# ocramz/rp-tree

Measured on AMD Instinct MI355X. Metric: forest-build vectors/s (1000000 x 128 dense f64, 32 trees; projection mode mfma = RPT_PROJ_MFMA, the API default RPT_PROJ_AUTO on f64 data is the exact-order kernel timed in `other_projection_mode`); kNN queries/s and recall@10 in `knn` / `recall_at_10`, higher is better.
Workload: dtype f64; 1 GPU; C2: 1000000 x 128 f64 two-Gaussian mixture, 32-tree forest, minLeaf 128, maxDepth 13, pnz 0.4746, k=10, 10000 queries; trees sharded 32/GPU, X replicated; projection_mode=mfma

## Files before the change

rp-tree_amd/csrc/split.hip:

```cpp
#include <algorithm>
#include <chrono>
#include <cmath>
#include <cstdio>
#include <cstdlib>
#include <functional>
#include <limits>
#include <list>

#include "common.h"
#include "codes.h"

extern "C" __device__ unsigned int __ockl_median3_u32(unsigned int, unsigned int, unsigned int);

namespace rpt {
namespace {

constexpr int kSmallCap = 4096;
constexpr int kNB = 1024;
constexpr int kSample = 1024;
constexpr int kDelta = 80;
constexpr int kChunk = 4096;
constexpr int kPad = 0x7fffffff;

template <class TK>
// ... 3004 lines not shown
  if (!(kmin < kmax)) return false;
  const double inv = 1024.0 / ((double)kmax - (double)kmin);
  auto sub_of = [&](TK k) -> int {
    const int b = (int)(((double)k - (double)kmin) * inv);
    return b > 1023 ? 1023 : b;
  };
  for (int i = tid; i < cMid; i += 256) atomicAdd(&sel_hist[sub_of(skey[i])], 1);
  __syncthreads();
  const int kk = a.nh - a.cL;
  if (wave == 0) {
    int c[16], tot = 0;
#pragma unroll
    for (int q = 0; q < 16; ++q) {
      c[q] = sel_hist[lane * 16 + q];
      tot += c[q];
    }
    int inc = tot;
    for (int o = 1; o < 64; o <<= 1) {
      const int p = __shfl_up(inc, o);
      if (lane >= o) inc += p;
    }
    int run = inc - tot;
    if (kk >= run && kk < inc) {
#pragma unroll
      for (int q = 0; q < 16; ++q) {
        if (kk >= run && kk < run + c[q]) {
          sel_misc[0] = lane * 16 + q;
          sel_misc[1] = run;
          sel_misc[2] = c[q];
        }
        run += c[q];
      }
    }
  }
  __syncthreads();
  const int sstar = sel_misc[0], below = sel_misc[1], mc = sel_misc[2];
  if (mc > 128) return false;
  unsigned long long lowmax = 0ULL, highmin = ~0ULL;
  for (int i = tid; i < cMid; i += 256) {
    const TK k = skey[i];
    const int sb = sub_of(k);
    if (sb == sstar) {
      sel_cand[atomicAdd(&sel_misc[3], 1)] = i;
    } else {
      const unsigned long long o = ord_of(k);
      if (sb < sstar) lowmax = o > lowmax ? o : lowmax;
      else highmin = o < highmin ? o : highmin;
    }
  }
  for (int o = 32; o > 0; o >>= 1) {
    const unsigned long long p = __shfl_xor(lowmax, o), q = __shfl_xor(highmin, o);
    lowmax = p > lowmax ? p : lowmax;
    highmin = q < highmin ? q : highmin;
  }
  __syncthreads();
  if (lane == 0) {
    sel_red[wave] = lowmax;
    sel_red[4 + wave] = highmin;
  }
  __syncthreads();
  uint16_t* no = A.node_of + (int64_t)t * N;
  unsigned long long mn[2] = {~0ULL, ~0ULL}, mx[2] = {0ULL, 0ULL};
  const bool feed_next = A.has_next && cMid * 4 >= a.n;
  auto place = [&](int id, int side) {
    no[id] = (uint16_t)(2 * j + side);
    if (feed_next) {
      const unsigned long long o = ord_of(mid_next_key(A, t, id));
      mn[side] = o < mn[side] ? o : mn[side];
      mx[side] = o > mx[side] ? o : mx[side];
    }
  };
  if (wave == 0) {
    for (int w = 0; w < 4; ++w) {
      lowmax = sel_red[w] > lowmax ? sel_red[w] : lowmax;
      highmin = sel_red[4 + w] < highmin ? sel_red[4 + w] : highmin;
    }
    Keys<TK> K{A.P + (int64_t)t * A.L * N, N, A.level, nullptr};
    TK k[2];
    int id[2];
#pragma unroll
    for (int r = 0; r < 2; ++r) {
      const int q = r * 64 + lane;
      const int i = q < mc ? sel_cand[q] : -1;
      id[r] = i >= 0 ? sid[i] : kPad;
      k[r] = i >= 0 ? skey[i] : pos_inf<TK>();
    }
    wave_bitonic_fast<TK, 2>(k, id, K);
    const int n = a.n, nh = a.nh;
    const int il = nh > 0 ? nh - 1 : 0, ih = nh + 1 < n ? nh + 1 : n - 1;
    const int ql = il - a.cL, qh = ih - a.cL;
    TK vthr = (TK)0, vlo = (TK)0, vhi = (TK)0;
    int have = 0;
#pragma unroll
    for (int r = 0; r < 2; ++r) {
      const int q = below + r * 64 + lane;
      if (r * 64 + lane < mc) {
        place(id[r], q >= kk);
        if (q == kk) {
          vthr = k[r];
          have |= 1;
        }
        if (q == ql) {
          vlo = k[r];
          have |= 2;
        }
        if (q == qh) {
          vhi = k[r];
          have |= 4;
        }
      }
    }
    const unsigned long long b1 = __ballot(have & 1), b2 = __ballot(have & 2), b4 = __ballot(have & 4);
    const TK tthr = __shfl(vthr, __ffsll((long long)b1) - 1);
    TK tlo, thi;
    if (b2) tlo = __shfl(vlo, __ffsll((long long)b2) - 1);
    else if (ql < 0) tlo = ord_to(a.maxL, TK());
    else tlo = ord_to(lowmax, TK());
    if (b4) thi = __shfl(vhi, __ffsll((long long)b4) - 1);
    else if (qh >= cMid) thi = ord_to(a.minR, TK());
    else thi = ord_to(highmin, TK());
    if (lane == 0) {
      const int64_t h = (int64_t)t * A.nodes + A.heap0 + j;
      A.thr[h] = (double)tthr;
      A.mglo[h] = (double)tlo;
      A.mghi[h] = (double)thi;
      if (nh > 0 && !(tlo < tthr)) atomicAdd(A.tie_count, 1ULL);
    }
  }
  for (int i = tid; i < cMid; i += 256) {
    const int sb = sub_of(skey[i]);
    if (sb != sstar) place(sid[i], sb > sstar);
  }
  if (feed_next) {
    for (int sd = 0; sd < 2; ++sd) {
      unsigned long long x = mn[sd], y = mx[sd];
      for (int o = 32; o > 0; o >>= 1) {
        const unsigned long long p = __shfl_xor(x, o), q = __shfl_xor(y, o);
        x = p < x ? p : x;
        y = q > y ? q : y;
      }
      if (lane == 0) {
        if (x != ~0ULL) atomicMin(&A.cmin_next[(int64_t)t * 2 * M + 2 * j + sd], x);
        if (y != 0ULL) atomicMax(&A.cmax_next[(int64_t)t * 2 * M + 2 * j + sd], y);
      }
    }
  }
  return true;
}

constexpr int kMidWaveLds = 512;

template <class TK>
__global__ __launch_bounds__(256) void stream_mid(const MidArgs<TK> A, int npb, int wave_max,
                                                  int use_select ) {
  extern __shared__ __attribute__((aligned(16))) unsigned char smem[];
  __shared__ int sbig[4];
  const int w = threadIdx.x >> 6, lane = threadIdx.x & 63, t = blockIdx.y;
  const int jw = blockIdx.x * npb + w;
  int big = 0;
  if (w < npb && jw < A.M) {
    const SNode<TK> a = A.nd[(int64_t)t * A.M + jw];
    if (a.cMid > wave_max) {
      if (npb > 1 && a.cMid <= kMidWaveLds)
        mid_lds_path<TK, true>(A, a, t, jw, smem + (size_t)w * kMidWaveLds * (sizeof(TK) + 4));
      else
        big = a.cMid <= kSmallCap;
    } else if (a.cMid > 0) {
      mid_wave_path<TK>(A, a, t, jw, lane);
    }
  }
  if (lane == 0) sbig[w] = big;
  __syncthreads();
  for (int q = 0; q < npb; ++q) {
    if (!sbig[q]) continue;
    const int j = blockIdx.x * npb + q;
    const SNode<TK> a = A.nd[(int64_t)t * A.M + j];
    if (use_select && mid_select_path<TK>(A, a, t, j, smem)) {
      __syncthreads();
      continue;
    }
    __syncthreads();
    mid_lds_path<TK, false>(A, a, t, j, smem);
    __syncthreads();
  }
}

constexpr int kPermChunk = 8192;
template <class TK>
__global__ __launch_bounds__(kStreamThreads) void stream_to_perm(
    const uint16_t* __restrict__ node_of, int64_t N, int levels, int64_t per,
    unsigned int* __restrict__ gcur, int32_t* __restrict__ perm,
    const unsigned int* __restrict__ abort) {
  constexpr int EPT = kPermChunk / kStreamThreads;
  __shared__ unsigned int cnt[2 * kStreamMaxNodes];
  __shared__ int gb[2 * kStreamMaxNodes], noff[2 * kStreamMaxNodes];
  __shared__ int sid[kPermChunk];
  __shared__ unsigned short sj[kPermChunk];
  __shared__ unsigned int wsum[kStreamThreads / 64];
  if (*abort) return;
  const int t = blockIdx.y;
  const int M = 1 << levels;
  const int lane = threadIdx.x & 63, wave = threadIdx.x >> 6;
  const uint16_t* no = node_of + (int64_t)t * N;
  int32_t* pm = perm + (int64_t)t * N;
  const int64_t i0 = (int64_t)blockIdx.x * per, i1 = i0 + per < N ? i0 + per : N;
  for (int j = threadIdx.x; j < M; j += kStreamThreads) {
    int64_t off = 0, n = N;
    for (int b = levels - 1; b >= 0; --b) {
      const int64_t nh = n >> 1;
      if ((j >> b) & 1) {
        off += nh;
        n -= nh;
      } else {
        n = nh;
      }
    }
    noff[j] = (int)off;
  }
  for (int64_t c0 = i0; c0 < i1; c0 += kPermChunk) {
    const int cn = (int)(i1 - c0 < kPermChunk ? i1 - c0 : kPermChunk);
    for (int j = threadIdx.x; j < M; j += kStreamThreads) cnt[j] = 0;
    __syncthreads();
    unsigned int pk[EPT];
#pragma unroll
    for (int e = 0; e < EPT; ++e) {
      const int k = e * kStreamThreads + threadIdx.x;
      pk[e] = 0xffffffffu;
      if (k < cn) {
        const unsigned int j = no[c0 + k];
        pk[e] = (j << 16) | atomicAdd(&cnt[j], 1u);
      }
    }
    __syncthreads();
    unsigned int v0 = 0, v1 = 0;
    const int j0 = 2 * threadIdx.x, j1 = j0 + 1;
    if (j0 < M) v0 = cnt[j0];
    if (j1 < M) v1 = cnt[j1];
    unsigned int inc = v0 + v1;
    for (int o = 1; o < 64; o <<= 1) {
      const unsigned int u = __shfl_up(inc, o);
      if (lane >= o) inc += u;
    }
    if (lane == 63) wsum[wave] = inc;
    __syncthreads();
    unsigned int pre = inc - (v0 + v1);
    for (int w = 0; w < wave; ++w) pre += wsum[w];
    if (j0 < M) {
      cnt[j0] = pre;
      gb[j0] = v0 ? noff[j0] + (int)atomicAdd(&gcur[(int64_t)t * M + j0], v0) - (int)pre : 0;
    }
    if (j1 < M) {
      cnt[j1] = pre + v0;
      gb[j1] = v1 ? noff[j1] + (int)atomicAdd(&gcur[(int64_t)t * M + j1], v1) - (int)(pre + v0) : 0;
    }
    __syncthreads();
#pragma unroll
    for (int e = 0; e < EPT; ++e)
      if (pk[e] != 0xffffffffu) {
        const unsigned int j = pk[e] >> 16, r = pk[e] & 0xffffu;
        const int sl = (int)(cnt[j] + r);
        sid[sl] = (int)(c0 + e * kStreamThreads + threadIdx.x);
        sj[sl] = (unsigned short)j;
      }
    __syncthreads();
    for (int k = threadIdx.x; k < cn; k += kStreamThreads) pm[gb[sj[k]] + k] = sid[k];
    __syncthreads();
  }
}

__device__ inline double sample_value(double v) { return v; }
__device__ inline double sample_value(float v) { return (double)v; }
__device__ inline double sample_value(uint16_t v) {
  return (double)__uint_as_float((unsigned int)v << 16);
}
template <class TIn, class TK>
__global__ __launch_bounds__(256) void sample_range_kernel(const TIn* __restrict__ X, int64_t stride,
                                                           int S, int d, const double* __restrict__ R,
                                                           int C, int L, int Lc,
                                                           unsigned long long* __restrict__ mm) {
  constexpr int CG = 16, KCH = 128;
  __shared__ __attribute__((aligned(16))) double rl[KCH * CG];
  const int c0 = blockIdx.x * CG;
  const int si = blockIdx.y * 256 + threadIdx.x;
  const bool live = si < S;
  const TIn* xr = X + (int64_t)(live ? si : 0) * stride * d;
  double acc[CG];
#pragma unroll
  for (int c = 0; c < CG; ++c) acc[c] = 0.0;
  for (int k0 = 0; k0 < d; k0 += KCH) {
    const int kn = d - k0 < KCH ? d - k0 : KCH;
    __syncthreads();
    for (int i = threadIdx.x; i < kn * CG; i += 256) {
      const int c = i / kn, k = i % kn;
      rl[k * CG + c] = c0 + c < C ? R[(int64_t)(c0 + c) * d + k0 + k] : 0.0;
    }
    __syncthreads();
    int k = 0;
    for (; k + 16 <= kn; k += 16) {
      TIn xv[16];
#pragma unroll
      for (int u = 0; u < 16; ++u) xv[u] = xr[k0 + k + u];
#pragma unroll
      for (int u = 0; u < 16; ++u) {
        const double x = sample_value(xv[u]);
#pragma unroll
        for (int c = 0; c < CG; ++c) acc[c] = __builtin_fma(x, rl[(k + u) * CG + c], acc[c]);
      }
    }
    for (; k < kn; ++k) {
      const double x = sample_value(xr[k0 + k]);
#pragma unroll
      for (int c = 0; c < CG; ++c) acc[c] = __builtin_fma(x, rl[k * CG + c], acc[c]);
    }
  }
  unsigned long long mn = ~0ULL, mx = 0ULL;
#pragma unroll
  for (int c = 0; c < CG; ++c) {
    const TK v = (TK)acc[c];
    if (live && c0 + c < C && (c0 + c) % L < Lc && v == v) {
      const unsigned long long o = ord_of(v);
      mn = o < mn ? o : mn;
      mx = o > mx ? o : mx;
    }
  }
  for (int o = 32; o > 0; o >>= 1) {
    const unsigned long long a = __shfl_xor(mn, o), b = __shfl_xor(mx, o);
    mn = a < mn ? a : mn;
    mx = b > mx ? b : mx;
  }
  if ((threadIdx.x & 63) == 0 && mn <= mx) {
    atomicMin(&mm[0], mn);
    atomicMax(&mm[1], mx);
  }
}

template <class TK>
__global__ __launch_bounds__(256) void pcode_range_kernel(const TK* __restrict__ P, int64_t N, int L,
                                                          int Lc, unsigned long long* mm) {
  const int c = blockIdx.x;
  if (c % L >= Lc) return;
  const TK* col = P + (int64_t)c * N;
  const int64_t m = N < 4096 ? N : 4096;
  unsigned long long mn = ~0ULL, mx = 0ULL;
  for (int64_t i = threadIdx.x; i < m; i += 256) {
    const unsigned long long o = ord_of(col[i * N / m]);
    mn = o < mn ? o : mn;
    mx = o > mx ? o : mx;
  }
  for (int o = 32; o > 0; o >>= 1) {
    const unsigned long long a = __shfl_xor(mn, o), b = __shfl_xor(mx, o);
    mn = a < mn ? a : mn;
    mx = b > mx ? b : mx;
  }
  if ((threadIdx.x & 63) == 0) {
    atomicMin(mm, mn);
    atomicMax(mm + 1, mx);
  }
}

template <class TK>
__global__ __launch_bounds__(256) void pcode_kernel(const TK* __restrict__ P, int64_t N, int L, int Lc,
                                                    const unsigned long long* __restrict__ mm,
                                                    uint16_t* __restrict__ codes) {
  const int c = blockIdx.y;
  if (c % L >= Lc) return;
  const CodeGeo<TK> g = code_geo<TK>(mm[0], mm[1]);
  const TK* col = P + (int64_t)c * N;
  uint16_t* out = codes + (int64_t)c * N;
  const int64_t n8 = N / 8;
  for (int64_t i = (int64_t)blockIdx.x * 256 + threadIdx.x; i < n8; i += (int64_t)gridDim.x * 256) {
    struct alignas(16) V8 { uint16_t v[8]; } o;
#pragma unroll
    for (int e = 0; e < 8; ++e) o.v[e] = code_of(col[i * 8 + e], g);
    *reinterpret_cast<V8*>(out + i * 8) = o;
  }
  if (blockIdx.x == 0)
    for (int64_t i = n8 * 8 + threadIdx.x; i < N; i += 256) out[i] = code_of(col[i], g);
}

__global__ void build_init_kernel(double* thr, double* mglo, double* mghi, int64_t n,
                                  unsigned long long* counters , unsigned int* sflags ) {
  const double nan = __longlong_as_double(0x7ff8000000000000LL);
  for (int64_t i = blockIdx.x * (int64_t)blockDim.x + threadIdx.x; i < n;
       i += (int64_t)gridDim.x * blockDim.x) {
    thr[i] = nan;
    mglo[i] = nan;
    mghi[i] = nan;
  }
  if (blockIdx.x == 0 && threadIdx.x < 2) counters[threadIdx.x] = 0ULL;
  if (blockIdx.x == 0 && threadIdx.x < 4) sflags[threadIdx.x] = 0u;
}

__global__ void stream_init_kernel(unsigned long long* cmin, unsigned long long* cmax, int T,
                                   unsigned int* poolcur, int npool) {
  for (int i = blockIdx.x * blockDim.x + threadIdx.x; i < T; i += gridDim.x * blockDim.x) {
    cmin[i] = ~0ULL;
    cmax[i] = 0ULL;
  }
  for (int i = blockIdx.x * blockDim.x + threadIdx.x; i < npool; i += gridDim.x * blockDim.x)
    poolcur[i] = 0u;
}

struct GSeg {
  int64_t off;
  int32_t n;
  int32_t t;
  int32_t heap;
  int32_t nh_rel, il_rel, ih_rel;
};

template <class TK>
__global__ __launch_bounds__(256) void gsort_chunk_kernel(int32_t* buf, int64_t N, const TK* P,
                                                          int L, int level,
                                                          const GSeg* __restrict__ gs,
                                                          const int32_t* tb) {
  extern __shared__ __attribute__((aligned(16))) unsigned char smem[];
  const GSeg g = gs[blockIdx.y];
  const int64_t c0 = (int64_t)blockIdx.x * kSmallCap;
  if (c0 >= g.n) return;
  const int n = (int)((g.n - c0) < kSmallCap ? (g.n - c0) : kSmallCap);
  const int np = next_pow2(n);
  TK* skey = reinterpret_cast<TK*>(smem);
  int* sid = reinterpret_cast<int*>(smem + (size_t)np * sizeof(TK));
  Keys<TK> K{P + (int64_t)g.t * L * N, N, level, tb ? tb + (int64_t)g.t * N : nullptr};
  int32_t* s = buf + g.off + c0;
  for (int i = threadIdx.x; i < np; i += blockDim.x) {
    if (i < n) {
      const int id = s[i];
      sid[i] = id;
      skey[i] = K.key(id);
    } else {
      sid[i] = kPad;
      skey[i] = pos_inf<TK>();
    }
  }
  __syncthreads();
  lds_bitonic(skey, sid, np, K);
  for (int i = threadIdx.x; i < n; i += blockDim.x) s[i] = sid[i];
}

template <class TK>
__global__ __launch_bounds__(256) void gsort_merge_kernel(const int32_t* __restrict__ in,
                                                          int32_t* __restrict__ out, int64_t N,
                                                          const TK* P, int L, int level,
                                                          const GSeg* __restrict__ gs, int64_t w,
                                                          const int32_t* tb) {
  const GSeg g = gs[blockIdx.y];
  const int64_t i = (int64_t)blockIdx.x * 256 + threadIdx.x;
  if (i >= g.n) return;
  Keys<TK> K{P + (int64_t)g.t * L * N, N, level, tb ? tb + (int64_t)g.t * N : nullptr};
  const int32_t* s = in + g.off;
  const int id = s[i];
  const int64_t run = i / w, pair0 = (run & ~1LL) * w;
  const bool in_a = (run & 1) == 0;
  const int64_t o0 = in_a ? pair0 + w : pair0;
  int64_t olen = g.n - o0;
  if (olen > w) olen = w;
  int64_t rank = 0;
  if (olen > 0) {
    const TK key = K.key(id);
    int64_t lo = 0, hi = olen;
    while (lo < hi) {
      const int64_t mid = (lo + hi) >> 1;
      const int oid = s[o0 + mid];
      if (K.less(K.key(oid), oid, key, id)) lo = mid + 1;
      else hi = mid;
    }
    rank = lo;
  }
  const int64_t own = in_a ? i - pair0 : i - (pair0 + w);
  out[g.off + pair0 + own + rank] = id;
}

__global__ void gsort_copy_kernel(const int32_t* __restrict__ in, int32_t* __restrict__ out,
                                  const GSeg* __restrict__ gs) {
  const GSeg g = gs[blockIdx.y];
  const int64_t i = (int64_t)blockIdx.x * 256 + threadIdx.x;
  if (i < g.n) out[g.off + i] = in[g.off + i];
}

template <class TK>
__global__ void gsort_emit_kernel(const int32_t* __restrict__ buf, int64_t N, const TK* P, int L,
                                  int level, const GSeg* __restrict__ gs, int G,
                                  const NodeAux* aux_of , const int* aux_idx,
                                  double* thr, double* mglo, double* mghi, int64_t nodes,
                                  unsigned long long* tie_count) {
  const int gi = blockIdx.x * blockDim.x + threadIdx.x;
  if (gi >= G) return;
  const GSeg g = gs[gi];
  if (g.heap < 0) return;
  const TK* Pl = P + ((int64_t)g.t * L + level) * N;
  const int64_t h = (int64_t)g.t * nodes + g.heap;
  const TK vthr = Pl[buf[g.off + g.nh_rel]];
  TK vlo, vhi;
  if (g.il_rel >= 0) vlo = Pl[buf[g.off + g.il_rel]];
  else vlo = ord_to(aux_of[aux_idx[gi]].maxL, TK());
  if (g.ih_rel >= 0) vhi = Pl[buf[g.off + g.ih_rel]];
  else vhi = ord_to(aux_of[aux_idx[gi]].minR, TK());
  thr[h] = (double)vthr;
  mglo[h] = (double)vlo;
  mghi[h] = (double)vhi;
  if (!(vlo < vthr)) atomicAdd(tie_count, 1ULL);
}

template <class TK>
int32_t gsort(rpt_ctx* ctx, int32_t* buf, int32_t* tmp, int64_t N, const TK* P, int L, int level,
              const std::vector<GSeg>& list, DevBuf<GSeg>& dlist, const int32_t* tb) {
  if (list.empty()) return RPT_OK;
  RPT_TRY(dlist.alloc(list.size()));
  RPT_HIP(hipMemcpyAsync(dlist.p, list.data(), list.size() * sizeof(GSeg), hipMemcpyHostToDevice,
                         ctx->stream));
  RPT_HIP(stream_sync(ctx->stream));
  int64_t nmax = 0;
  for (const GSeg& g : list) nmax = g.n > nmax ? g.n : nmax;
  const unsigned G = (unsigned)list.size();
  const size_t smem = (size_t)kSmallCap * (sizeof(TK) + 4);
  hipLaunchKernelGGL(gsort_chunk_kernel<TK>, dim3((unsigned)((nmax + kSmallCap - 1) / kSmallCap), G),
                     dim3(256), smem, ctx->stream, buf, N, P, L, level, dlist.p, tb);
  int32_t* a = buf;
  int32_t* b = tmp;
  for (int64_t w = kSmallCap; w < nmax; w *= 2) {
    hipLaunchKernelGGL(gsort_merge_kernel<TK>, dim3((unsigned)((nmax + 255) / 256), G), dim3(256),
                       0, ctx->stream, a, b, N, P, L, level, dlist.p, w, tb);
    std::swap(a, b);
  }
  if (a != buf)
    hipLaunchKernelGGL(gsort_copy_kernel, dim3((unsigned)((nmax + 255) / 256), G), dim3(256), 0,
                       ctx->stream, a, buf, dlist.p);
  RPT_HIP(hipGetLastError());
  return RPT_OK;
}

static double now_ms() {
  return std::chrono::duration<double, std::milli>(std::chrono::steady_clock::now().time_since_epoch()).count();
}
#define HT(label) do { if (ctx->opt.debug_host) { (void)stream_sync(ctx->stream); double t__ = now_ms(); fprintf(stderr, "host %-28s %8.3f ms\n", label, t__ - ht_last); ht_last = t__; } } while (0)

template <class TK>
int32_t build_forest_t(rpt_ctx* ctx, const rpt_dataset* ds, rpt_forest* f, int32_t mode,
                       bool no_stream = false) {
  double ht_last = now_ms();
  const int64_t N = f->n;
  const int T = f->T, L = f->L;
  hipStream_t st = ctx->stream;
  f->mode = mode;
  ctx->last_csub_redo = ctx->last_csub_bad = 0;

  int Lused = 0;
  {
    int64_t n = N;
    for (int l = 0; l < L; ++l) {
      if (n > (int64_t)f->min_leaf) Lused = l + 1;
      n -= n / 2;
    }
  }
  DevBuf<unsigned long long> counters;
  DevBuf<unsigned int> sflags;
  RPT_TRY(counters.alloc(2));
  RPT_TRY(sflags.alloc(4));
  hipLaunchKernelGGL(build_init_kernel, dim3(256), dim3(256), 0, st, f->thr.p, f->mglo.p, f->mghi.p,
                     (int64_t)T * f->nodes, counters.p, sflags.p);
  if (N == 0) return RPT_OK;
  if (Lused == 0) {
    hipLaunchKernelGGL(iota_kernel, dim3(1024), dim3(256), 0, st, f->perm.p, N, T);
    RPT_HIP(hipGetLastError());
    return RPT_OK;
  }

  RPT_TRY(f->proj.alloc((size_t)T * L * N * sizeof(TK)));
  TK* P = reinterpret_cast<TK*>(f->proj.p);
  const int stream_cap = ctx->opt.stream_maxnodes > 0
                             ? (int)(ctx->opt.stream_maxnodes < kStreamMaxNodes ? ctx->opt.stream_maxnodes
                                                                                : kStreamMaxNodes)
                             : (N / 1024 > kSmallCap ? 1024 : 512);
  int Lc = 0;
  if (N >= 2048 && !no_stream && !ctx->opt.no_stream) {
    int64_t nmin = N;
    while (Lc < Lused && nmin > (int64_t)f->min_leaf && (1 << Lc) <= stream_cap) {
      ++Lc;
      nmin /= 2;
    }
  }
  int Lcodes = Lc;
  if (Lc > 0 && !ctx->opt.no_csub) {
    int64_t nmax = N, nmin = N;
    for (int l = 0; l < Lc; ++l) {
      nmax -= nmax / 2;
      nmin /= 2;
    }
    if (nmax > kWCap && nmax <= kCsCap) {
      int r = 0;
      while (nmax > kWCap) {
        nmax -= nmax / 2;
        nmin /= 2;
        ++r;
      }
      if (r <= kCsMaxR && Lc + r < L && nmin > (int64_t)f->min_leaf) Lcodes = Lc + r;
    }
  }
  DevBuf<uint16_t> codes;
  DevBuf<unsigned long long> code_mm;
  uint16_t* Cd = nullptr;
  const bool codes_wanted = Lc > 0 && Lused == L && N >= ((int64_t)1 << 17) && !ctx->opt.no_codes;
  if (codes_wanted && !project_writes_codes(ctx, ds, mode) && !ctx->opt.no_pcodes &&
      (N % 8) == 0) {
    RPT_TRY(project_columns(ctx, ds, f->R.p, T * L, mode, P));
    RPT_TRY(code_mm.alloc(2));
    RPT_TRY(codes.alloc((size_t)T * L * N));
    ProfScope ps(ctx, RPT_PROF_SPLIT);
    hipLaunchKernelGGL(stream_init_kernel, dim3(1), dim3(64), 0, st, code_mm.p, code_mm.p + 1, 1,
                       (unsigned int*)nullptr, 0);
    hipLaunchKernelGGL(pcode_range_kernel<TK>, dim3((unsigned)(T * L)), dim3(256), 0, st,
                       (const TK*)P, N, L, Lcodes, code_mm.p);
    const unsigned pb = (unsigned)std::min<int64_t>((N / 8 + 255) / 256, (int64_t)ctx->n_cu * 4);
    hipLaunchKernelGGL(pcode_kernel<TK>, dim3(pb > 0 ? pb : 1, (unsigned)(T * L)), dim3(256), 0, st,
                       (const TK*)P, N, L, Lcodes, (const unsigned long long*)code_mm.p, codes.p);
    RPT_HIP(hipGetLastError());
    Cd = codes.p;
  } else if (codes_wanted && project_writes_codes(ctx, ds, mode)) {
    constexpr int S = 4096;
    const int C = T * L;
    RPT_TRY(code_mm.alloc(2));
    hipLaunchKernelGGL(stream_init_kernel, dim3(1), dim3(64), 0, st, code_mm.p, code_mm.p + 1, 1,
                       (unsigned int*)nullptr, 0);
    const int64_t stride = N / S;
    const dim3 sgrid((unsigned)((C + 15) / 16), (unsigned)((S + 255) / 256));
    if (ds->dtype == RPT_F64)
      hipLaunchKernelGGL((sample_range_kernel<double, TK>), sgrid, dim3(256), 0, st,
                         (const double*)ds->X, stride, S, f->d, f->R.p, C, L, Lcodes, code_mm.p);
    else if (ds->dtype == RPT_F32)
      hipLaunchKernelGGL((sample_range_kernel<float, TK>), sgrid, dim3(256), 0, st,
                         (const float*)ds->X, stride, S, f->d, f->R.p, C, L, Lcodes, code_mm.p);
    else
      hipLaunchKernelGGL((sample_range_kernel<uint16_t, TK>), sgrid, dim3(256), 0, st,
                         (const uint16_t*)ds->X, stride, S, f->d, f->R.p, C, L, Lcodes, code_mm.p);
    RPT_TRY(codes.alloc((size_t)T * L * N));
    CodeOut co;
    co.codes = codes.p;
    co.mm = code_mm.p;
    co.ld = N;
    co.L = L;
    co.Lc = Lcodes;
    bool written = false;
    RPT_TRY(project_columns(ctx, ds, f->R.p, C, mode, P, &co, &written));
    if (written) Cd = codes.p;
    else codes.release();
  } else if (Lused == L) {
    RPT_TRY(project_columns(ctx, ds, f->R.p, T * L, mode, P));
  } else {
    for (int t = 0; t < T; ++t)
      RPT_TRY(project_columns(ctx, ds, f->R.p + (int64_t)t * L * f->d, Lused, mode,
                              P + (int64_t)t * L * N));
  }

  std::vector<Node> topo;
  enumerate_topology(N, L, f->min_leaf, topo);
  std::vector<std::vector<Seg>> splits((size_t)Lused), leaves((size_t)Lused + 1);
  for (const Node& nd : topo) {
    Seg s{nd.off, (int32_t)nd.n, nd.leaf ? -1 : (int32_t)nd.heap};
    if (nd.leaf) leaves[(size_t)nd.level].push_back(s);
    else splits[(size_t)nd.level].push_back(s);
  }

  HT("projection");
  DevBuf<int32_t> bufA, bufB;
  DevBuf<TK> Kst;
  RPT_TRY(bufA.alloc((size_t)T * N));
  RPT_TRY(bufB.alloc((size_t)T * N));
  size_t Smax = 1, SbigMax = 0;
  for (auto& v : splits) {
    Smax = v.size() > Smax ? v.size() : Smax;
    if (!v.empty() && v[0].n > kSmallCap) SbigMax = v.size() > SbigMax ? v.size() : SbigMax;
  }
  DevBuf<Seg> dsegs, dsegs2;
  DevBuf<BinInfo<TK>> bins;
  DevBuf<NodeAux> aux;
  DevBuf<unsigned int> hist, bigflags;
  DevBuf<GSeg> dglist;
  DevBuf<unsigned int> ovf;
  bool have_big = false;
  for (auto& v : splits)
    for (const Seg& s : v) have_big = have_big || s.n > kSmallCap;
  if (have_big) {
    RPT_TRY(Kst.alloc((size_t)T * N));
    size_t sb = 0;
    for (auto& v : splits) {
      size_t c = 0;
      for (const Seg& s : v) c += s.n > kSmallCap;
      sb = c > sb ? c : sb;
    }
    RPT_TRY(bins.alloc((size_t)T * sb));
    RPT_TRY(aux.alloc((size_t)T * sb));
    RPT_TRY(hist.alloc((size_t)T * sb * kNB));
    RPT_TRY(bigflags.alloc((size_t)T * sb));
    RPT_HIP(hipMemsetAsync(hist.p, 0, (size_t)T * sb * kNB * 4, st));
  }

  int32_t* F = f->perm.p;
  unsigned long long* dbgbuf = nullptr;
  DevBuf<unsigned long long> dbgdev;
  if (ctx->opt.debug_stamps) {
    RPT_TRY(dbgdev.alloc(256));
    RPT_HIP(hipMemsetAsync(dbgdev.p, 0, 256 * 8, st));
    dbgbuf = dbgdev.p;
  }
  unsigned long long* tie_count = counters.p;
  unsigned int* big_count = reinterpret_cast<unsigned int*>(counters.p + 1);

  auto upload = [&](const std::vector<Seg>& v, DevBuf<Seg>& d) -> int32_t {
    RPT_TRY(d.ensure(v.size()));
    return upload_async(ctx, d.p, v.data(), v.size() * sizeof(Seg));
  };

  struct PNode {
    Seg seg;
    int buf;
  };
  std::vector<std::vector<PNode>> pending((size_t)Lused + kRmax + 1);
  int32_t* bufs[2] = {bufA.p, bufB.p};
  bool stream_unchecked = false;
  auto stream_aborted = [&](bool* aborted) -> int32_t {
    *aborted = false;
    if (!stream_unchecked) return RPT_OK;
    unsigned int v = 0;
    RPT_HIP(hipMemcpy(&v, sflags.p, 4, hipMemcpyDeviceToHost));
    stream_unchecked = false;
    *aborted = v != 0;
    return RPT_OK;
  };
  HT("alloc work buffers");
  int Lstream = 0;
  if (N >= 2048 && !no_stream && !ctx->opt.no_stream)
  {
    int max_nodes = ctx->opt.stream_maxnodes > 0 ? (int)ctx->opt.stream_maxnodes
                                                 : (N / 1024 > kSmallCap ? 1024 : 512);
    if (max_nodes > kStreamMaxNodes) max_nodes = kStreamMaxNodes;
    while (Lstream < Lused && splits[(size_t)Lstream].size() == ((size_t)1 << Lstream) &&
           (1 << Lstream) <= max_nodes)
      ++Lstream;
  }
  int streamed = 0;
  if (Lstream > 0) {
    DevBuf<uint16_t> node_of;
    DevBuf<unsigned int> part, poolcur, gcur, totals;
    DevBuf<SNode<TK>> snodes;
    DevBuf<unsigned long long> mm[4];
    const int64_t min_per = ctx->opt.stream_minper > 0 ? ctx->opt.stream_minper : 32768;
    int64_t nblk = (2 * (int64_t)ctx->n_cu + T - 1) / T;
    if (nblk > (N + min_per - 1) / min_per) nblk = (N + min_per - 1) / min_per;
    if (nblk < (N + 65519) / 65520) nblk = (N + 65519) / 65520;
    if (nblk < 1) nblk = 1;
    const int64_t per = (((N + nblk - 1) / nblk) + 7) & ~(int64_t)7;
    const dim3 sgrid((unsigned)nblk, (unsigned)T);
    const int64_t afac = ctx->opt.tune0 > 0 ? ctx->opt.tune0 : ((Cd && Lstream <= Lc) ? 2 : 1);
    int64_t nblkA = (afac * (int64_t)ctx->n_cu + T - 1) / T;
    if (nblkA > (N + 8191) / 8192) nblkA = (N + 8191) / 8192;
    if (nblkA < 1) nblkA = 1;
    const int64_t perA = (((N + nblkA - 1) / nblkA) + 7) & ~(int64_t)7;
    const dim3 agrid((unsigned)nblkA, (unsigned)T);
    RPT_TRY(node_of.alloc((size_t)T * N));
    RPT_TRY(part.alloc((size_t)T * nblk * (kStreamBins / 2)));
    RPT_TRY(poolcur.alloc((size_t)T * Lstream));
    RPT_TRY(snodes.alloc((size_t)T * kStreamMaxNodes));
    for (auto& b : mm) RPT_TRY(b.alloc((size_t)T * 2 * kStreamMaxNodes));
    RPT_HIP(hipMemsetAsync(node_of.p, 0, (size_t)T * N * 2, st));
    unsigned long long *cmin = mm[0].p, *cmax = mm[1].p, *cminN = mm[2].p, *cmaxN = mm[3].p;
    hipLaunchKernelGGL(stream_init_kernel, dim3(4), dim3(256), 0, st, cmin, cmax, T, poolcur.p,
                       T * Lstream);
    const uint16_t* Cs = (Cd && Lstream <= Lc) ? Cd : nullptr;
    hipLaunchKernelGGL(stream_minmax0<TK>, sgrid, dim3(kStreamThreads), 0, st, P, Cs, N, L, per, cmin,
                       cmax);
    HT("stream alloc+minmax0");
    int32_t* pool = bufB.p;
    DevBuf<TK> poolkey;
    RPT_TRY(poolkey.alloc((size_t)T * N));
    const int wave_max = ctx->opt.no_wmid ? 0 : 128;
    const int use_select = ctx->opt.no_midselect ? 0 : 1;
    const int64_t big_node = ctx->opt.stream_big_node > 0 ? ctx->opt.stream_big_node
                                                          : ((int64_t)1 << 21);
    {
      ProfScope ps(ctx, RPT_PROF_SPLIT);
      for (int level = 0; level < Lstream; ++level) {
        const int M = 1 << level;
        const int has_next = level + 1 < Lstream ? 1 : 0;
        const int B = stream_bins(M, N >> level, big_node);
        hipLaunchKernelGGL(stream_hist<TK>, sgrid, dim3(kStreamThreads), 0, st, P, Cs, node_of.p, N,
                           L, level, M, B, per, cmin, cmax, part.p);
        unsigned int* pc = poolcur.p + (size_t)level * T;
#define RPT_PICK(BPT, G)                                                                       \
  hipLaunchKernelGGL((stream_pick<TK, BPT, G>), dim3((unsigned)((M + 256 / G - 1) / (256 / G)), \
                                                      (unsigned)T),                            \
                     dim3(256), 0, st, N, level, M, (int)nblk, part.p, cmin, cmax, snodes.p, pc, \
                     cminN, cmaxN, sflags.p, Cs ? 1 : 0)
        switch (B) {
          case 4096: RPT_PICK(16, 256); break;
          case 2048: RPT_PICK(8, 256); break;
          case 1024: RPT_PICK(8, 128); break;
          case 512: RPT_PICK(8, 64); break;
          case 256: RPT_PICK(8, 32); break;
          case 128: RPT_PICK(8, 16); break;
          case 64: RPT_PICK(8, 8); break;
          case 32: RPT_PICK(8, 4); break;
          default: {
            RPT_TRY(totals.ensure((size_t)T * kStreamBins));
            hipLaunchKernelGGL(stream_pick_sum, dim3((unsigned)((M * B / 2 + 255) / 256), (unsigned)T),
                               dim3(256), 0, st, M * B / 2, (int)nblk, part.p, totals.p);
            hipLaunchKernelGGL(stream_pick_big<TK>, dim3((unsigned)M, (unsigned)T), dim3(256), 0, st,
                               N, level, M, B, totals.p, cmin, cmax, snodes.p, pc, cminN, cmaxN,
                               sflags.p, Cs ? 1 : 0);
          }
        }
#undef RPT_PICK
        if (Cs)
          hipLaunchKernelGGL((stream_assign<TK, true>), agrid, dim3(kStreamThreads), 0, st, P, Cs, node_of.p, N,
                             L, level, M, B, perA, has_next, snodes.p, pool, poolkey.p, cminN, cmaxN);
        else
          hipLaunchKernelGGL((stream_assign<TK, false>), agrid, dim3(kStreamThreads), 0, st, P, Cs, node_of.p, N,
                             L, level, M, B, perA, has_next, snodes.p, pool, poolkey.p, cminN, cmaxN);
        const size_t smem = (size_t)kSmallCap * (sizeof(TK) + 4);
        const int npb = M >= 16 ? 4 : 1;
        MidArgs<TK> ma{P,     Cs,   node_of.p, N,     L,        level,    M,
                       has_next, snodes.p, pool, poolkey.p, cminN, cmaxN, (int64_t)M - 1, f->nodes,
                       f->thr.p, f->mglo.p, f->mghi.p, tie_count};
        hipLaunchKernelGGL(stream_mid<TK>, dim3((unsigned)((M + npb - 1) / npb), (unsigned)T),
                           dim3(256), smem, st, ma, npb, wave_max, use_select);
        std::swap(cmin, cminN);
        std::swap(cmax, cmaxN);
      }
      RPT_HIP(hipGetLastError());
      streamed = Lstream;
      stream_unchecked = true;
    }
    HT("stream levels");
    {
      ProfScope ps(ctx, RPT_PROF_SPLIT);
      const int M = 1 << streamed;
      std::vector<Seg> lvl((size_t)M);
      for (int j = 0; j < M; ++j) {
        int64_t off = 0, n = N;
        for (int b = streamed - 1; b >= 0; --b) {
          const int64_t nh = n / 2;
          if ((j >> b) & 1) {
            off += nh;
            n -= nh;
          } else {
            n = nh;
          }
        }
        lvl[(size_t)j] = Seg{off, (int32_t)n, (int32_t)(M - 1 + j)};
      }
      RPT_TRY(gcur.alloc((size_t)T * M));
      RPT_HIP(hipMemsetAsync(gcur.p, 0, (size_t)T * M * 4, st));
      hipLaunchKernelGGL(stream_to_perm<TK>, sgrid, dim3(kStreamThreads), 0, st, node_of.p, N,
                         streamed, per, gcur.p, bufA.p, sflags.p);
      RPT_HIP(hipGetLastError());
      std::vector<Seg> lsmall;
      std::vector<GSeg> lbig;
      std::vector<Seg> lbig_copy;
      for (const Seg& c : lvl) {
        if (!is_leaf(streamed, c.n, L, f->min_leaf)) {
          pending[(size_t)streamed].push_back(PNode{c, 0});
        } else if (c.n <= kSmallCap) {
          lsmall.push_back(Seg{c.off, c.n, -1});
        } else {
          lbig_copy.push_back(Seg{c.off, c.n, -1});
          for (int t = 0; t < T; ++t)
            lbig.push_back(GSeg{(int64_t)t * N + c.off, c.n, t, -1, -1, -1, -1});
        }
      }
      if (!lsmall.empty() || !lbig.empty()) {
        RPT_HIP(ctx_sync(ctx));
        bool aborted = false;
        RPT_TRY(stream_aborted(&aborted));
        if (aborted) return build_forest_t<TK>(ctx, ds, f, mode, true);
      }
      if (!lsmall.empty()) {
        RPT_TRY(upload(lsmall, dsegs));
        int nm = 0;
        for (const Seg& sgm : lsmall) nm = sgm.n > nm ? sgm.n : nm;
        const size_t sm2 = (size_t)next_pow2(nm) * (sizeof(TK) + 4);
        hipLaunchKernelGGL(small_sort_kernel<TK>, dim3((unsigned)lsmall.size(), T), dim3(256), sm2,
                           st, bufA.p, F, N, P, L, streamed - 1, dsegs.p, (const int32_t*)nullptr,
                           f->thr.p, f->mglo.p, f->mghi.p, f->nodes, tie_count);
      }
      if (!lbig.empty()) {
        RPT_TRY(gsort<TK>(ctx, bufA.p, bufB.p, N, P, L, streamed - 1, lbig, dglist, nullptr));
        RPT_TRY(upload(lbig_copy, dsegs));
        hipLaunchKernelGGL(copy_segs_kernel, dim3((unsigned)lbig_copy.size(), T), dim3(256), 0, st,
                           bufA.p, F, N, dsegs.p);
      }
      RPT_HIP(hipGetLastError());
    }
  }
  HT("stream to_perm + free");
  if (stream_unchecked) {
    bool all_wave = !ctx->opt.no_wsub;
    for (const PNode& pn : pending[(size_t)streamed]) all_wave = all_wave && pn.seg.n <= kWCap;
    if (!all_wave) {
      RPT_HIP(ctx_sync(ctx));
      bool aborted = false;
      RPT_TRY(stream_aborted(&aborted));
      if (aborted) return build_forest_t<TK>(ctx, ds, f, mode, true);
    }
  }
  if (streamed == 0) {
    hipLaunchKernelGGL(iota_kernel, dim3(1024), dim3(256), 0, st, bufA.p, N, T);
    if (!splits[0].empty()) pending[0].push_back(PNode{splits[0][0], 0});
  }
  std::function<void(const Seg&, int, int, int, std::vector<Seg>&)> descend =
      [&](const Seg& sgm, int level, int depth, int want, std::vector<Seg>& out) {
        if (is_leaf(level, sgm.n, L, f->min_leaf)) return;
        if (depth == want) {
          out.push_back(sgm);
          return;
        }
        const int nh = sgm.n / 2;
        descend(Seg{sgm.off, nh, 2 * sgm.heap + 1}, level + 1, depth + 1, want, out);
        descend(Seg{sgm.off + nh, sgm.n - nh, 2 * sgm.heap + 2}, level + 1, depth + 1, want, out);
      };

  DevBuf<double> wgeo;
  DevBuf<unsigned long long> wpacked;
  DevBuf<unsigned long long> cpacked;
  DevBuf<unsigned int> csflags;
  DevBuf<Seg> dsegs_cs;
  struct Deferred {
    int level = 0, b = 0;
    std::vector<Seg> nodes;
    DevBuf<unsigned int> flags;
  };
  std::list<Deferred> deferred;

  for (int level = 0; level < Lused; ++level) {
    for (int b = 0; b < 2; ++b) {
      std::vector<Seg> small, big, mid;
      int cs_r = 0;
      if (Cd && !ctx->opt.no_csub) {
        int nmax = 0, nmin = 0x7fffffff;
        for (const PNode& pn : pending[(size_t)level])
          if (pn.buf == b && pn.seg.n > kWCap && pn.seg.n <= kCsCap) {
            nmax = pn.seg.n > nmax ? pn.seg.n : nmax;
            nmin = pn.seg.n < nmin ? pn.seg.n : nmin;
          }
        if (nmax > 0) {
          int r = 0;
          while (nmax > kWCap) {
            nmax -= nmax / 2;
            nmin /= 2;
            ++r;
          }
          if (r <= kCsMaxR && level + r <= Lcodes && !is_leaf(level + r, nmin, L, f->min_leaf)) cs_r = r;
        }
      }
      for (const PNode& pn : pending[(size_t)level])
        if (pn.buf == b) {
          if (cs_r > 0 && pn.seg.n > kWCap && pn.seg.n <= kCsCap) mid.push_back(pn.seg);
          else (pn.seg.n > kSmallCap ? big : small).push_back(pn.seg);
        }
      if (small.empty() && big.empty() && mid.empty()) continue;
      ProfScope ps(ctx, RPT_PROF_SPLIT);
      int32_t* cur = bufs[b];
      int32_t* nxt = bufs[1 - b];
      if (!mid.empty()) {
        const unsigned S = (unsigned)mid.size();
        RPT_TRY(upload(mid, dsegs_cs));
        RPT_TRY(csflags.ensure((size_t)S + 1));
        RPT_HIP(hipMemsetAsync(csflags.p, 0, ((size_t)S + 1) * 4, st));
        RPT_TRY(cpacked.ensure((size_t)T * N));
        const unsigned pb = (unsigned)std::min<int64_t>((N + 1023) / 1024, (int64_t)ctx->n_cu * 8);
        hipLaunchKernelGGL(cpack_kernel, dim3(pb, T), dim3(256), 0, st, (const uint16_t*)Cd, N, L, level,
                           cs_r, cpacked.p);
        int csmax = 0;
        for (const Seg& sgm : mid) csmax = sgm.n > csmax ? sgm.n : csmax;
#define RPT_CSUB(E)                                                                              \
  hipLaunchKernelGGL((csub_kernel<TK, E>), dim3(S, T), dim3(kCsThreads), 0, st, cur, nxt, N, P,  \
                     (const unsigned long long*)cpacked.p, L, level, cs_r, dsegs_cs.p, f->thr.p, \
                     f->mglo.p, f->mghi.p, f->nodes, tie_count, csflags.p)
        if (csmax <= 8 * kCsThreads) RPT_CSUB(8);
// ... 715 lines not shown
```

Before: 230.9 million vectors/s.

## Register-tile sample range GEMM and size stream_mid LDS by node cap

Rewrites the sampled projection-range kernel as a 64x64 register-tiled GEMM with swizzled LDS tiles for both X and R, a register prefetch of the next k-chunk, and a block-level min/max reduction with guarded atomics. It also sizes stream_mid's dynamic shared memory to the largest possible node size at the current level instead of always reserving kSmallCap, passing that cap to the kernel. The goal is to raise data reuse in the range estimate and allow more resident blocks in stream_mid at deep levels. The tiled kernel uses more registers, and the smaller LDS reservation relies on the node-size bound holding.

```diff
diff --git a/rp-tree_amd/csrc/split.hip b/rp-tree_amd/csrc/split.hip
--- a/rp-tree_amd/csrc/split.hip
+++ b/rp-tree_amd/csrc/split.hip
@@ -3180,7 +3180,8 @@
 
 template <class TK>
 __global__ __launch_bounds__(256) void stream_mid(const MidArgs<TK> A, int npb, int wave_max,
-                                                  int use_select ) {
+                                                  int use_select ,
+                                                  int cap ) {
   extern __shared__ __attribute__((aligned(16))) unsigned char smem[];
   __shared__ int sbig[4];
   const int w = threadIdx.x >> 6, lane = threadIdx.x & 63, t = blockIdx.y;
@@ -3192,7 +3193,7 @@
       if (npb > 1 && a.cMid <= kMidWaveLds)
         mid_lds_path<TK, true>(A, a, t, jw, smem + (size_t)w * kMidWaveLds * (sizeof(TK) + 4));
       else
-        big = a.cMid <= kSmallCap;
+        big = a.cMid <= cap;
     } else if (a.cMid > 0) {
       mid_wave_path<TK>(A, a, t, jw, lane);
     }
@@ -3301,64 +3302,98 @@
 __device__ inline double sample_value(uint16_t v) {
   return (double)__uint_as_float((unsigned int)v << 16);
 }
+constexpr int kSrRows = 64, kSrCols = 64, kSrK = 64;
+__device__ inline int sr_at(int r, int k) { return r * kSrK + (k ^ ((r & 15) << 1)); }
 template <class TIn, class TK>
 __global__ __launch_bounds__(256) void sample_range_kernel(const TIn* __restrict__ X, int64_t stride,
                                                            int S, int d, const double* __restrict__ R,
                                                            int C, int L, int Lc,
                                                            unsigned long long* __restrict__ mm) {
-  constexpr int CG = 16, KCH = 128;
-  __shared__ __attribute__((aligned(16))) double rl[KCH * CG];
-  const int c0 = blockIdx.x * CG;
-  const int si = blockIdx.y * 256 + threadIdx.x;
-  const bool live = si < S;
-  const TIn* xr = X + (int64_t)(live ? si : 0) * stride * d;
-  double acc[CG];
-#pragma unroll
-  for (int c = 0; c < CG; ++c) acc[c] = 0.0;
-  for (int k0 = 0; k0 < d; k0 += KCH) {
-    const int kn = d - k0 < KCH ? d - k0 : KCH;
+  __shared__ __attribute__((aligned(16))) double xs[kSrRows * kSrK], rs[kSrCols * kSrK];
+  typedef double dbl2 __attribute__((ext_vector_type(2)));
+  constexpr int NX = kSrRows * kSrK / 256, NR = kSrCols * kSrK / 256;
+  const int c0 = blockIdx.x * kSrCols, s0 = blockIdx.y * kSrRows;
+  const int tx = threadIdx.x & 15, ty = threadIdx.x >> 4;
+  const int lk = threadIdx.x & (kSrK - 1), lr = threadIdx.x / kSrK;
+  TIn xg[NX];
+  double rg[NR];
+  auto fetch = [&](int k0) {
+    const bool kin = k0 + lk < d;
+#pragma unroll
+    for (int e = 0; e < NX; ++e) {
+      const int si = s0 + lr + e * (256 / kSrK);
+      xg[e] = kin && si < S ? X[(int64_t)si * stride * d + k0 + lk] : TIn(0);
+    }
+#pragma unroll
+    for (int e = 0; e < NR; ++e) {
+      const int c = c0 + lr + e * (256 / kSrK);
+      rg[e] = kin && c < C ? R[(int64_t)c * d + k0 + lk] : 0.0;
+    }
+  };
+  double acc[4][4];
+#pragma unroll
+  for (int i = 0; i < 4; ++i)
+#pragma unroll
+    for (int j = 0; j < 4; ++j) acc[i][j] = 0.0;
+  fetch(0);
+  for (int k0 = 0; k0 < d; k0 += kSrK) {
     __syncthreads();
-    for (int i = threadIdx.x; i < kn * CG; i += 256) {
-      const int c = i / kn, k = i % kn;
-      rl[k * CG + c] = c0 + c < C ? R[(int64_t)(c0 + c) * d + k0 + k] : 0.0;
-    }
+#pragma unroll
+    for (int e = 0; e < NX; ++e) xs[sr_at(lr + e * (256 / kSrK), lk)] = sample_value(xg[e]);
+#pragma unroll
+    for (int e = 0; e < NR; ++e) rs[sr_at(lr + e * (256 / kSrK), lk)] = rg[e];
     __syncthreads();
-    int k = 0;
-    for (; k + 16 <= kn; k += 16) {
-      TIn xv[16];
-#pragma unroll
-      for (int u = 0; u < 16; ++u) xv[u] = xr[k0 + k + u];
-#pragma unroll
-      for (int u = 0; u < 16; ++u) {
-        const double x = sample_value(xv[u]);
-#pragma unroll
-        for (int c = 0; c < CG; ++c) acc[c] = __builtin_fma(x, rl[(k + u) * CG + c], acc[c]);
-      }
-    }
-    for (; k < kn; ++k) {
-      const double x = sample_value(xr[k0 + k]);
-#pragma unroll
-      for (int c = 0; c < CG; ++c) acc[c] = __builtin_fma(x, rl[k * CG + c], acc[c]);
+    if (k0 + kSrK < d) fetch(k0 + kSrK);
+    const int kn = d - k0 < kSrK ? (d - k0 + 1) & ~1 : kSrK;
+    for (int k = 0; k < kn; k += 2) {
+      dbl2 xv[4], rv[4];
+#pragma unroll
+      for (int i = 0; i < 4; ++i) {
+        xv[i] = *reinterpret_cast<const dbl2*>(xs + sr_at(ty + 16 * i, k));
+        rv[i] = *reinterpret_cast<const dbl2*>(rs + sr_at(tx + 16 * i, k));
+      }
+#pragma unroll
+      for (int i = 0; i < 4; ++i)
+#pragma unroll
+        for (int j = 0; j < 4; ++j) {
+          acc[i][j] = __builtin_fma(xv[i][0], rv[j][0], acc[i][j]);
+          acc[i][j] = __builtin_fma(xv[i][1], rv[j][1], acc[i][j]);
+        }
     }
   }
   unsigned long long mn = ~0ULL, mx = 0ULL;
 #pragma unroll
-  for (int c = 0; c < CG; ++c) {
-    const TK v = (TK)acc[c];
-    if (live && c0 + c < C && (c0 + c) % L < Lc && v == v) {
-      const unsigned long long o = ord_of(v);
-      mn = o < mn ? o : mn;
-      mx = o > mx ? o : mx;
-    }
-  }
+  for (int i = 0; i < 4; ++i)
+#pragma unroll
+    for (int j = 0; j < 4; ++j) {
+      const int si = s0 + ty + 16 * i, c = c0 + tx + 16 * j;
+      const TK v = (TK)acc[i][j];
+      if (si < S && c < C && c % L < Lc && v == v) {
+        const unsigned long long o = ord_of(v);
+        mn = o < mn ? o : mn;
+        mx = o > mx ? o : mx;
+      }
+    }
   for (int o = 32; o > 0; o >>= 1) {
     const unsigned long long a = __shfl_xor(mn, o), b = __shfl_xor(mx, o);
     mn = a < mn ? a : mn;
     mx = b > mx ? b : mx;
   }
-  if ((threadIdx.x & 63) == 0 && mn <= mx) {
-    atomicMin(&mm[0], mn);
-    atomicMax(&mm[1], mx);
+  __shared__ unsigned long long red[8];
+  if ((threadIdx.x & 63) == 0) {
+    red[threadIdx.x >> 6] = mn;
+    red[4 + (threadIdx.x >> 6)] = mx;
+  }
+  __syncthreads();
+  if (threadIdx.x == 0) {
+    for (int w = 0; w < 4; ++w) {
+      mn = red[w] < mn ? red[w] : mn;
+      mx = red[4 + w] > mx ? red[4 + w] : mx;
+    }
+    if (mn <= mx) {
+      if (mn < __atomic_load_n(&mm[0], __ATOMIC_RELAXED)) atomicMin(&mm[0], mn);
+      if (mx > __atomic_load_n(&mm[1], __ATOMIC_RELAXED)) atomicMax(&mm[1], mx);
+    }
   }
 }
 
@@ -3652,7 +3687,7 @@
     hipLaunchKernelGGL(stream_init_kernel, dim3(1), dim3(64), 0, st, code_mm.p, code_mm.p + 1, 1,
                        (unsigned int*)nullptr, 0);
     const int64_t stride = N / S;
-    const dim3 sgrid((unsigned)((C + 15) / 16), (unsigned)((S + 255) / 256));
+    const dim3 sgrid((unsigned)((C + kSrCols - 1) / kSrCols), (unsigned)((S + kSrRows - 1) / kSrRows));
     if (ds->dtype == RPT_F64)
       hipLaunchKernelGGL((sample_range_kernel<double, TK>), sgrid, dim3(256), 0, st,
                          (const double*)ds->X, stride, S, f->d, f->R.p, C, L, Lcodes, code_mm.p);
@@ -3845,13 +3880,16 @@
         else
           hipLaunchKernelGGL((stream_assign<TK, false>), agrid, dim3(kStreamThreads), 0, st, P, Cs, node_of.p, N,
                              L, level, M, B, perA, has_next, snodes.p, pool, poolkey.p, cminN, cmaxN);
-        const size_t smem = (size_t)kSmallCap * (sizeof(TK) + 4);
         const int npb = M >= 16 ? 4 : 1;
+        int mid_cap = kSmallCap;
+        if (((N - 1) >> level) + 1 < (int64_t)kSmallCap) mid_cap = next_pow2((int)(((N - 1) >> level) + 1));
+        if (npb > 1 && mid_cap < npb * kMidWaveLds) mid_cap = npb * kMidWaveLds;
+        const size_t smem = (size_t)mid_cap * (sizeof(TK) + 4);
         MidArgs<TK> ma{P,     Cs,   node_of.p, N,     L,        level,    M,
                        has_next, snodes.p, pool, poolkey.p, cminN, cmaxN, (int64_t)M - 1, f->nodes,
                        f->thr.p, f->mglo.p, f->mghi.p, tie_count};
         hipLaunchKernelGGL(stream_mid<TK>, dim3((unsigned)((M + npb - 1) / npb), (unsigned)T),
-                           dim3(256), smem, st, ma, npb, wave_max, use_select);
+                           dim3(256), smem, st, ma, npb, wave_max, use_select, mid_cap);
         std::swap(cmin, cminN);
         std::swap(cmax, cmaxN);
       }
```

After: 237.4 million vectors/s (median of 6 runs). 1.03x the previous value.
